# michal7kw/scRNA_seq_QAnnealing_Clustering

Measured on AMD Instinct MI355X. Metric: spin-flip updates/sec (node) + best QUBO energy vs neal, PBMC3k SNN, higher is better.
Workload: dtype f32

## Files before the change

scrna_seq_qannealing_clustering_amd/csrc/sparse_pair_kernels.hip:

```cpp
#include "mi_sa_device.h"

namespace mi_sa_impl {

namespace {

typedef _Float16 half_t;

#ifdef MI_K2P_PROFILE
#define K2P_TICK(var) do { asm volatile("s_waitcnt lgkmcnt(0)" ::: "memory"); const unsigned long long now_ = __builtin_amdgcn_s_memtime(); var += now_ - tick_; tick_ = now_; } while (0)
#else
#define K2P_TICK(var) do { } while (0)
#endif

__device__ __forceinline__ float half_lo(uint32_t w) { return (float)__builtin_bit_cast(half_t, (uint16_t)w); }
__device__ __forceinline__ float half_hi(uint32_t w) { return (float)__builtin_bit_cast(half_t, (uint16_t)(w >> 16)); }

template <int D, bool TW, bool WGT = false, int RW = D, int N16 = 0>
__global__ void __launch_bounds__(TW ? 128 : 64, TW ? 1 : 2) k_anneal_csr_rank1_pair(EllArgs a)
{
    static_assert(RW > D - 4 && RW <= D, "trimmed rows drop part of the last group of four only");
    static_assert(N16 == 0 || !WGT, "the weighted form keeps the 32-bit packing");
    static_assert(N16 != 2 || (TW && D == 16), "the pipelined unpack lives in the threshold-wavefront form's gather window");
    extern __shared__ __attribute__((aligned(16))) char lds[];
    const int lane = threadIdx.x & 63;
    const int pair = blockIdx.x;
    const int rA = 2 * pair, rB = 2 * pair + 1;
    if (rA >= a.R) return;
    const bool liveB = rB < a.R;
    const uint32_t gidA = a.replica_offset + (uint32_t)rA, gidB = gidA + 1u;
    const int n = a.n, slots = a.slots;
    const uint8_t *init = static_cast<const uint8_t *>(a.init);
    uint32_t *cell = reinterpret_cast<uint32_t *>(lds);
    const uint32_t ring_lane = (uint32_t)slots * 256u + (uint32_t)lane * 8u;

    if constexpr (TW) {
        if (__builtin_amdgcn_readfirstlane((int)(threadIdx.x >> 6)) == 1) {
            uint32_t wa[4], wb[4];
            uint32_t buf = 0;
            for (int s = 0; s < a.num_sweeps; ++s) {
                float TA, TB;
                if (a.temps_per_replica) {
                    TA = __int_as_float(__builtin_amdgcn_readfirstlane(__float_as_int(a.temps[rA])));
                    TB = __int_as_float(__builtin_amdgcn_readfirstlane(__float_as_int(a.temps[liveB ? rB : rA])));
                } else {
                    TA = TB = __int_as_float(__builtin_amdgcn_readfirstlane(__float_as_int(a.temps[s])));
                }
                const uint32_t sw = (uint32_t)s + a.sweep_offset;
#pragma unroll 1
                for (int t = 0; t < slots; t += 4) {
#ifdef MI_K2P_DBG_NOPROD
                    for (int c = 0; c < 4; ++c) wa[c] = wb[c] = (uint32_t)(t + c) * 0x9E3779B9u + lane * 77u;
#else
                    philox4x32_10((uint32_t)((t >> 2) * 64 + lane), sw, gidA, 0u, a.seed_lo, a.seed_hi, wa);
                    philox4x32_10((uint32_t)((t >> 2) * 64 + lane), sw, gidB, 0u, a.seed_lo, a.seed_hi, wb);
#endif
                    const uint32_t at = ring_lane + buf;
#pragma unroll
                    for (int c = 0; c < 4; ++c) {
                        const f32x2_t thr = neglog_u2(wa[c], wb[c]) * f32x2_t{TA, TB};
                        asm volatile("ds_write_b64 %0, %1 offset:%2" :: "v"(at), "v"(thr), "n"(c * 512) : "memory");
                    }
                    buf ^= 2048u;
                    asm volatile("s_waitcnt lgkmcnt(0)" ::: "memory");
                    __builtin_amdgcn_s_barrier();
                }
            }
            return;
        }
    }

    const int wslot = WGT ? a.wslot : -1;
    const int wl = wslot >= 0 ? a.wgt[lane] : 0;
    int SA = 0, SB = 0;
    for (int tg = 0; tg * 4 < slots; ++tg) {
        uint32_t wa[4] = {0u, 0u, 0u, 0u}, wb[4] = {0u, 0u, 0u, 0u};
        if (!init) {
            philox4x32_10((uint32_t)(tg * 64 + lane), 0u, gidA, 1u, a.seed_lo, a.seed_hi, wa);
            philox4x32_10((uint32_t)(tg * 64 + lane), 0u, gidB, 1u, a.seed_lo, a.seed_hi, wb);
        }
#pragma unroll
        for (int c = 0; c < 4; ++c) {
            const int t = 4 * tg + c;
            if (t >= slots) break;
            const int i = t * 64 + lane;
            bool xa, xb;
            const bool real = i < n && a.lin[i] < INFINITY;
            if (init) {
                xa = real && init[(size_t)rA * n + i] != 0;
                xb = real && liveB && init[(size_t)rB * n + i] != 0;
            } else {
                xa = real && (wa[c] >> 31);
                xb = real && (wb[c] >> 31);
            }
            cell[i] = (xa ? 0x3c00u : 0u) | (xb ? 0x3c000000u : 0u);
            if (WGT && t == wslot) {
                SA += (int)wave_sum_i64(xa ? (long long)wl : 0ll);
                SB += (int)wave_sum_i64(xb ? (long long)wl : 0ll);
            } else {
                SA += __popcll(__ballot(xa));
                SB += __popcll(__ballot(xb));
            }
        }
    }

    constexpr int G = D / 4;
    constexpr int LW = RW - 4 * (G - 1);
    constexpr int GC = N16 ? G / 2 : G;
    constexpr int SLOT_BYTES = N16 ? (GC + G) * 1024 : (G - 1) * 2048 + (LW == 3 ? 1792 : LW * 512);
    const __amdgpu_buffer_rsrc_t rs_adj = __builtin_amdgcn_make_buffer_rsrc(
        const_cast<uint4 *>(a.adj4), 0, slots * SLOT_BYTES, 0x00020000);
    const __amdgpu_buffer_rsrc_t rs_lin = __builtin_amdgcn_make_buffer_rsrc(
        const_cast<float *>(a.lin), 0, slots * 256, 0x00020000);
    struct SlotAdj { u32x4 col[GC]; u32x4 val[G]; uint32_t lin; };
    struct NbrPack { u32x4 w[GC]; };
    const int lane16 = lane * 16;
    auto fetch_block16 = [&](int t, int b) {
        const int tt = t < slots ? t : slots - 1;
        return __builtin_amdgcn_raw_buffer_load_b128(rs_adj, lane16 + (b & 3) * 1024, tt * SLOT_BYTES + (b >> 2) * 4096, 0);
    };
    auto fetch_nbr16 = [&](int t) {
        NbrPack q;
#pragma unroll
        for (int b = 0; b < GC; ++b) q.w[b] = fetch_block16(t, b);
        return q;
    };
    auto fetch_val16 = [&](int t) {
        SlotAdj p;
#pragma unroll
        for (int g = 0; g < G; ++g) p.val[g] = fetch_block16(t, GC + g);
        if constexpr (RW < D) p.lin = p.val[G - 1][3];
        else p.lin = __builtin_amdgcn_raw_buffer_load_b32(rs_lin, lane * 4, (t < slots ? t : slots - 1) * 256, 0);
        return p;
    };
    uint32_t m16 = 0xffffu;
    asm("" : "+s"(m16));
    auto unpack16 = [&](const u32x4 *w, int e) -> uint32_t {
        const uint32_t pw = w[e / 8][(e / 2) & 3];
        return (e & 1) ? pw >> 16 : (pw & m16);
    };
    uint32_t addr[16];
#ifdef MI_K2P_NOFETCH
    auto fetch_real = [&](int t) {
#else
    auto fetch_adj = [&](int t) {
#endif
        if constexpr (N16 != 0) {
            SlotAdj p = fetch_val16(t);
            const NbrPack q = fetch_nbr16(t);
#pragma unroll
            for (int b = 0; b < GC; ++b) p.col[b] = q.w[b];
            return p;
        }
        SlotAdj p;
        const int tt = t < slots ? t : slots - 1;
        const int soff = tt * SLOT_BYTES;
#pragma unroll
        for (int g = 0; g < G; ++g) {
            const int so = soff + (g / 2) * 4096, io = (g & 1) * 2048;
            if (LW == 4 || g < G - 1) {
                p.col[g] = __builtin_amdgcn_raw_buffer_load_b128(rs_adj, lane16 + io, so, 0);
                p.val[g] = __builtin_amdgcn_raw_buffer_load_b128(rs_adj, lane16 + io + 1024, so, 0);
            } else if constexpr (LW == 3) {
                p.col[g] = __builtin_amdgcn_raw_buffer_load_b128(rs_adj, lane16 + io, so, 0);
                const u32x2 v = __builtin_amdgcn_raw_buffer_load_b64(rs_adj, lane * 8 + io + 1024, so, 0);
                p.val[g] = u32x4{v.x, v.y, __builtin_amdgcn_raw_buffer_load_b32(rs_adj, lane * 4 + io + 1536, so, 0), 0u};
            } else if constexpr (LW == 2) {
                const u32x2 c = __builtin_amdgcn_raw_buffer_load_b64(rs_adj, lane * 8 + io, so, 0);
                const u32x2 v = __builtin_amdgcn_raw_buffer_load_b64(rs_adj, lane * 8 + io + 512, so, 0);
                p.col[g] = __builtin_shufflevector(c, c, 0, 1, -1, -1);
                p.val[g] = __builtin_shufflevector(v, v, 0, 1, -1, -1);
            } else {
                p.col[g][0] = __builtin_amdgcn_raw_buffer_load_b32(rs_adj, lane * 4 + io, so, 0);
                p.val[g][0] = __builtin_amdgcn_raw_buffer_load_b32(rs_adj, lane * 4 + io + 256, so, 0);
            }
        }
        if constexpr (LW == 3) p.lin = p.col[G - 1][3];
        else p.lin = __builtin_amdgcn_raw_buffer_load_b32(rs_lin, lane * 4, tt * 256, 0);
        return p;
    };
#ifdef MI_K2P_NOFETCH
    const SlotAdj adj0 = fetch_real(0);
    auto fetch_adj = [&](int) { return adj0; };
#endif

#ifdef MI_K2P_PROFILE
    unsigned long long tick_ = __builtin_amdgcn_s_memtime(), t_top = 0, t_gather = 0, t_sum = 0, t_rounds = 0, t_barrier = 0;
#endif
#ifndef MI_K2P_DBG_NOPRIO
    if constexpr (TW) __builtin_amdgcn_s_setprio(3);
#endif
    unsigned long long accepted = 0;
    uint32_t accA = 0, accB = 0;
    uint32_t wa[4] = {0u, 0u, 0u, 0u}, wb[4] = {0u, 0u, 0u, 0u};
    float TA = 1.0f, TB = 1.0f;
    const float cp = a.c_pair;
    uint32_t ring_buf = 0u;

    auto slot_body = [&](auto c_in_group, int t, const SlotAdj &cur, NbrPack &nxt, uint32_t wordA, uint32_t wordB) {
        constexpr int C = decltype(c_in_group)::value;
        const int i = t * 64 + lane;
        uint32_t own;
        float gA = __uint_as_float(cur.lin), gB = gA;
        float thrA = 0.0f, thrB = 0.0f;
        f32x2_t thr2 = {0.0f, 0.0f};
        uint32_t xiA = 0u, xiB = 0u, sgA = 0u, sgB = 0u;
        uint64_t XA = 0ull, XB = 0ull;
        f32x2_t cs = {0.0f, 0.0f}, csf = {0.0f, 0.0f};
        int ownA = 0, ownB = 0;
        auto own_terms = [&]() {
            xiA = (own >> 13) & 1u;
            xiB = own >> 29;
            XA = __ballot((own & 0xffffu) != 0u);
            XB = __ballot((own >> 16) != 0u);
            sgA = xiA << 31;
            sgB = xiB << 31;
            cs = f32x2_t{__uint_as_float(__float_as_uint(cp) ^ sgA), __uint_as_float(__float_as_uint(cp) ^ sgB)};
            ownA = SA - (int)xiA;
            ownB = SB - (int)xiB;
            csf = cs * f32x2_t{(float)ownA, (float)ownB};
        };
        K2P_TICK(t_top);
#pragma unroll
        for (int g0 = 0; g0 < G; g0 += 4) {
            constexpr int NK0 = RW < 16 ? RW : 16;
            const int NK = g0 == 0 ? NK0 : (RW - 4 * g0 < 16 ? RW - 4 * g0 : 16);
            uint32_t word[16];
            if (g0 == 0) asm volatile("ds_read_b32 %0, %1" : "=v"(own) : "v"(i * 4));
            if (g0 == 0 && TW) asm volatile("ds_read_b64 %0, %1 offset:%2" : "=v"(thr2) : "v"(ring_lane + ring_buf), "n"(C * 512));
#pragma unroll
            for (int k = 0; k < 16; ++k)
                if (k < NK)
#ifdef MI_K2P_DBG_LINEAR
                asm volatile("ds_read_b32 %0, %1" : "=v"(word[k]) : "v"((cur.col[g0 + k / 4][k & 3] & 0x3f00u) + lane * 4));
#else
                {
                    if constexpr (N16 == 2) asm volatile("ds_read_b32 %0, %1" : "=v"(word[k]) : "v"(addr[k]));
                    else if constexpr (N16 == 1) asm volatile("ds_read_b32 %0, %1" : "=v"(word[k]) : "v"(unpack16(cur.col, 4 * g0 + k)));
                    else
                asm volatile("ds_read_b32 %0, %1" : "=v"(word[k]) : "v"(cur.col[g0 + k / 4][k & 3]));
                }
#endif
            if (g0 == 0 && TW) {
                if constexpr (N16 == 2)
                    asm volatile("s_waitcnt lgkmcnt(%4)" : "+v"(own), "+v"(thr2), "+v"(nxt.w[0]), "+v"(nxt.w[1]) : "n"(NK0 < 15 ? NK0 : 15) : "memory");
                else
                asm volatile("s_waitcnt lgkmcnt(%2)" : "+v"(own), "+v"(thr2) : "n"(NK0 < 15 ? NK0 : 15) : "memory");
#ifndef MI_K2P_DBG_TERMS_AFTER
                own_terms();
#endif
                if constexpr (N16 == 2) {
#pragma unroll
                    for (int k = 0; k < NK0; ++k) {
                        addr[k] = unpack16(nxt.w, k);
                        asm volatile("" : "+v"(addr[k]));
                    }
                }
                asm volatile("s_waitcnt lgkmcnt(0)"
                             : "+v"(word[0]), "+v"(word[1]), "+v"(word[2]), "+v"(word[3]), "+v"(word[4]), "+v"(word[5]),
                               "+v"(word[6]), "+v"(word[7]), "+v"(word[8]), "+v"(word[9]), "+v"(word[10]), "+v"(word[11]),
                               "+v"(word[12]), "+v"(word[13]), "+v"(word[14]), "+v"(word[15]), "+v"(csf)
                             :: "memory");
                thrA = thr2.x;
                thrB = thr2.y;
            } else if (g0 == 0) {
                asm volatile("" : "+v"(wordA), "+v"(wordB));
                const f32x2_t thr = neglog_u2(wordA, wordB) * f32x2_t{TA, TB};
                thrA = thr.x;
                thrB = thr.y;
                asm volatile("s_waitcnt lgkmcnt(0)"
                             : "+v"(word[0]), "+v"(word[1]), "+v"(word[2]), "+v"(word[3]), "+v"(word[4]), "+v"(word[5]),
                               "+v"(word[6]), "+v"(word[7]), "+v"(word[8]), "+v"(word[9]), "+v"(word[10]), "+v"(word[11]),
                               "+v"(word[12]), "+v"(word[13]), "+v"(word[14]), "+v"(word[15]), "+v"(own), "+v"(thrA), "+v"(thrB)
                             :: "memory");
            } else {
                asm volatile("s_waitcnt lgkmcnt(0)"
                             : "+v"(word[0]), "+v"(word[1]), "+v"(word[2]), "+v"(word[3]), "+v"(word[4]), "+v"(word[5]),
                               "+v"(word[6]), "+v"(word[7]), "+v"(word[8]), "+v"(word[9]), "+v"(word[10]), "+v"(word[11]),
                               "+v"(word[12]), "+v"(word[13]), "+v"(word[14]), "+v"(word[15])
                             :: "memory");
            }
            K2P_TICK(t_gather);
#pragma unroll
            for (int k = 0; k < NK; ++k) {
                const float v = __uint_as_float(cur.val[g0 + k / 4][k & 3]);
                gA = __builtin_fmaf(v, half_lo(word[k]), gA);
                gB = __builtin_fmaf(v, half_hi(word[k]), gB);
            }
        }
#ifdef MI_K2P_DBG_TERMS_AFTER
        own_terms();
#else
        if constexpr (!TW) own_terms();
#endif
        if (WGT && t == wslot) {
            const uint64_t FA = weighted_slot_sweep(gA, thrA, wl, cp, xiA, SA, lane);
            const uint64_t FB = weighted_slot_sweep(gB, thrB, wl, cp, xiB, SB, lane);
            accA += (uint32_t)__popcll(FA);
            accB += (uint32_t)__popcll(FB);
            uint32_t fA, fB;
            asm("v_cndmask_b32 %0, 0, %1, %2" : "=v"(fA) : "v"(0x3c00u), "s"(FA));
            asm("v_cndmask_b32 %0, 0, %1, %2" : "=v"(fB) : "v"(0x3c000000u), "s"(FB));
            cell[i] = own ^ fA ^ fB;
            K2P_TICK(t_rounds);
            return;
        }
        const f32x2_t gs = {__uint_as_float(__float_as_uint(gA) ^ sgA), __uint_as_float(__float_as_uint(gB) ^ sgB)};
        f32x2_t de = gs + csf;
        bool mA = de.x < thrA, mB = de.y < thrB;
        uint64_t AA = __ballot(mA), AB = __ballot(mB);
        K2P_TICK(t_sum);
        if ((AA | AB) != 0ull) {
            const int baseA = ownA - (int)__builtin_amdgcn_mbcnt_hi((uint32_t)(XA >> 32), __builtin_amdgcn_mbcnt_lo((uint32_t)XA, 0u));
            const int baseB = ownB - (int)__builtin_amdgcn_mbcnt_hi((uint32_t)(XB >> 32), __builtin_amdgcn_mbcnt_lo((uint32_t)XB, 0u));
            uint64_t BA = AA ^ XA, BB = AB ^ XB;
#ifndef MI_K2P_DBG_NOROUNDS
#pragma nounroll
            for (;;) {
                const int sA = (int)__builtin_amdgcn_mbcnt_hi((uint32_t)(BA >> 32), __builtin_amdgcn_mbcnt_lo((uint32_t)BA, (uint32_t)baseA));
                const int sB = (int)__builtin_amdgcn_mbcnt_hi((uint32_t)(BB >> 32), __builtin_amdgcn_mbcnt_lo((uint32_t)BB, (uint32_t)baseB));
                de = gs + cs * f32x2_t{(float)sA, (float)sB};
                const uint64_t NBA = __ballot(de.x < thrA) ^ XA, NBB = __ballot(de.y < thrB) ^ XB;
                uint64_t d0 = NBA ^ BA, d1 = NBB ^ BB;
                asm("" : "+s"(d0), "+s"(d1));
                BA = NBA;
                BB = NBB;
                if ((d0 | d1) == 0ull) break;
            }
#endif
            AA = BA ^ XA;
            AB = BB ^ XB;
            SA += __popcll(BA) - __popcll(XA);
            SB += __popcll(BB) - __popcll(XB);
            accA += (uint32_t)__popcll(AA);
            accB += (uint32_t)__popcll(AB);
            uint32_t tA, tB;
            asm("v_cndmask_b32 %0, 0, %1, %2" : "=v"(tA) : "v"(0x3c00u), "s"(AA));
            asm("v_cndmask_b32 %0, 0, %1, %2" : "=v"(tB) : "v"(0x3c000000u), "s"(AB));
            cell[i] = own ^ tA ^ tB;
        }
        K2P_TICK(t_rounds);
    };

    using std::integral_constant;
    for (int s = 0; s < a.num_sweeps; ++s) {
        if constexpr (!TW) {
            if (a.temps_per_replica) {
                TA = __int_as_float(__builtin_amdgcn_readfirstlane(__float_as_int(a.temps[rA])));
                TB = __int_as_float(__builtin_amdgcn_readfirstlane(__float_as_int(a.temps[liveB ? rB : rA])));
            } else {
                TA = TB = __int_as_float(__builtin_amdgcn_readfirstlane(__float_as_int(a.temps[s])));
            }
        }
        const uint32_t sw = (uint32_t)s + a.sweep_offset;
        if constexpr (N16 == 2) {
            SlotAdj P = fetch_val16(0), Q;
            NbrPack NA = fetch_nbr16(0), NB;
#pragma unroll
            for (int k = 0; k < (RW < 16 ? RW : 16); ++k) addr[k] = unpack16(NA.w, k);
            NA = fetch_nbr16(1);
#pragma unroll 1
            for (int t = 0; t < slots; t += 4) {
                K2P_TICK(t_top);
                __builtin_amdgcn_s_barrier();
                K2P_TICK(t_barrier);
                Q = fetch_val16(t + 1);
                NB = fetch_nbr16(t + 2);
                slot_body(integral_constant<int, 0>{}, t, P, NA, wa[0], wb[0]);
                if (t + 1 < slots) {
                    P = fetch_val16(t + 2);
                    NA = fetch_nbr16(t + 3);
                    slot_body(integral_constant<int, 1>{}, t + 1, Q, NB, wa[1], wb[1]);
                    if (t + 2 < slots) {
                        Q = fetch_val16(t + 3);
                        NB = fetch_nbr16(t + 4);
                        slot_body(integral_constant<int, 2>{}, t + 2, P, NA, wa[2], wb[2]);
                        P = fetch_val16(t + 4);
                        NA = fetch_nbr16(t + 5);
                        if (t + 3 < slots) slot_body(integral_constant<int, 3>{}, t + 3, Q, NB, wa[3], wb[3]);
                    }
                }
                ring_buf ^= 2048u;
            }
        } else {
            NbrPack none;
            SlotAdj P = fetch_adj(0), Q;
    #pragma unroll 1
            for (int t = 0; t < slots; t += 4) {
                if constexpr (TW) {
                    K2P_TICK(t_top);
                    __builtin_amdgcn_s_barrier();
                    K2P_TICK(t_barrier);
                } else {
                    philox4x32_10((uint32_t)((t >> 2) * 64 + lane), sw, gidA, 0u, a.seed_lo, a.seed_hi, wa);
                    philox4x32_10((uint32_t)((t >> 2) * 64 + lane), sw, gidB, 0u, a.seed_lo, a.seed_hi, wb);
                }
                Q = fetch_adj(t + 1);
                slot_body(integral_constant<int, 0>{}, t, P, none, wa[0], wb[0]);
                if (t + 1 < slots) {
                    P = fetch_adj(t + 2);
                    slot_body(integral_constant<int, 1>{}, t + 1, Q, none, wa[1], wb[1]);
                    if (t + 2 < slots) {
                        Q = fetch_adj(t + 3);
                        slot_body(integral_constant<int, 2>{}, t + 2, P, none, wa[2], wb[2]);
                        P = fetch_adj(t + 4);
                        if (t + 3 < slots) slot_body(integral_constant<int, 3>{}, t + 3, Q, none, wa[3], wb[3]);
                    }
                }
                if constexpr (TW) ring_buf ^= 2048u;
            }
        }
        accepted += (unsigned long long)accA + (liveB ? (unsigned long long)accB : 0ull);
        accA = accB = 0;
    }

#pragma unroll 1
    for (int rep = 0; rep < 2; ++rep) {
        if (rep == 1 && !liveB) break;
        const int r = rep ? rB : rA;
        const int sh = rep ? 16 : 0;
        uint8_t *dst = static_cast<uint8_t *>(a.states) + (size_t)r * n;
        long long cnt = 0, cnt2 = 0;
        double e = 0.0;
        for (int t = 0; t < slots; ++t) {
            const int i = t * 64 + lane;
            const bool on = ((cell[i] >> sh) & 0xffffu) != 0u;
            if (i < n) dst[i] = (uint8_t)on;
            if (WGT && t == wslot) {
                cnt += wave_sum_i64(on ? (long long)wl : 0ll);
                cnt2 += wave_sum_i64(on ? (long long)wl * wl : 0ll);
            } else {
                const int c1 = __popcll(__ballot(on));
                cnt += c1;
                cnt2 += c1;
            }
            if (!on) continue;
            double acc = 0.0;
            for (int k = 0; k < D; ++k) {
                const size_t at = ((size_t)t * D + k) * 64 + lane;
                const uint32_t cc = a.ell_col[at];
                const double vv = a.ell_val64 ? a.ell_val64[at] : (double)a.ell_val[at];
                if (((cell[cc] >> sh) & 0xffffu) != 0u) acc += vv;
            }
            e += (a.lin64 ? a.lin64[i] : (double)a.lin[i]) + 0.5 * acc;
        }
        e = wave_sum_f64(e);
        if (lane == 0) {
            const double cp64 = a.ell_val64 ? a.c_pair64 : (double)a.c_pair;
            a.energy[r] = e + cp64 * 0.5 * ((double)cnt * (double)cnt - (double)cnt2) + a.offset;
        }
    }
    if (lane == 0) atomicAdd(&a.stats[1], accepted);
#ifdef MI_K2P_PROFILE
    if (lane == 0) {
        atomicAdd(&a.stats[8], t_top); atomicAdd(&a.stats[9], t_gather); atomicAdd(&a.stats[10], t_sum);
        atomicAdd(&a.stats[11], t_rounds); atomicAdd(&a.stats[12], t_barrier);
    }
#endif
}

}

int mi_launch_csr_rank1_pair(const EllArgs &a, const AnnealPlan &plan, hipStream_t st)
{
    if (!a.adj4) return fail(MI_EHIP, "csr_rank1 pair kernel: packed adjacency missing");
#ifdef MI_K2P_NOFETCH
    if (plan.nbr16) return fail(MI_EUNSUPPORTED, "the timing builds are arms of the 32-bit packing: set k2_nbr16 = 2");
#endif
    const int rw = plan.trim_rw ? plan.trim_rw : plan.D;
#define MI_K2P(D_, TW_, WGT_, RW_, N16_) \
    if (plan.D == D_ && plan.tw == TW_ && plan.weighted == WGT_ && rw == RW_ && (plan.nbr16 ? N16_ != 0 : N16_ == 0)) \
        return launch_planned(k_anneal_csr_rank1_pair<D_, TW_, WGT_, RW_, N16_>, a, plan, st);
    MI_K2P(16, true, true, 16, 0) MI_K2P(16, false, true, 16, 0)
    MI_K2P(16, true, false, 15, 2) MI_K2P(16, true, false, 14, 2) MI_K2P(16, true, false, 13, 2)
    MI_K2P(16, true, false, 15, 0) MI_K2P(16, true, false, 14, 0) MI_K2P(16, true, false, 13, 0)
    MI_K2P(16, true, false, 16, 2) MI_K2P(32, false, false, 32, 1)
    MI_K2P(16, true, false, 16, 0) MI_K2P(16, false, false, 16, 0) MI_K2P(32, false, false, 32, 0)
#undef MI_K2P
    return fail(MI_EUNSUPPORTED, "csr_rank1 pair kernel: slot-ELL width %d not built", a.D);
}

}
```

Baseline: 500.9 billion.

## Prefetch next slot's adjacency inside slot body and wrap prefetch across sweeps

In the 16-bit-packed pipelined path, the loads for upcoming slots are moved out of the outer loop and into each slot body via a callback, issued just before the LDS wait. The prefetch index wraps around to slot zero, so the pipeline carries into the next sweep without a per-sweep prologue refill. LDS cell and threshold-ring addresses become running base registers with immediate offsets, replacing per-slot address arithmetic. This adds state carried across sweeps and parity-dependent buffer swapping, which could be wrong for some slot counts.

```diff
diff --git a/scrna_seq_qannealing_clustering_amd/csrc/sparse_pair_kernels.hip b/scrna_seq_qannealing_clustering_amd/csrc/sparse_pair_kernels.hip
--- a/scrna_seq_qannealing_clustering_amd/csrc/sparse_pair_kernels.hip
+++ b/scrna_seq_qannealing_clustering_amd/csrc/sparse_pair_kernels.hip
@@ -114,9 +114,8 @@
     struct SlotAdj { u32x4 col[GC]; u32x4 val[G]; uint32_t lin; };
     struct NbrPack { u32x4 w[GC]; };
     const int lane16 = lane * 16;
-    auto fetch_block16 = [&](int t, int b) {
-        const int tt = t < slots ? t : slots - 1;
-        return __builtin_amdgcn_raw_buffer_load_b128(rs_adj, lane16 + (b & 3) * 1024, tt * SLOT_BYTES + (b >> 2) * 4096, 0);
+    auto fetch_block16 = [&](int w, int b) {
+        return __builtin_amdgcn_raw_buffer_load_b128(rs_adj, lane16 + (b & 3) * 1024, w * SLOT_BYTES + (b >> 2) * 4096, 0);
     };
     auto fetch_nbr16 = [&](int t) {
         NbrPack q;
@@ -129,7 +128,7 @@
 #pragma unroll
         for (int g = 0; g < G; ++g) p.val[g] = fetch_block16(t, GC + g);
         if constexpr (RW < D) p.lin = p.val[G - 1][3];
-        else p.lin = __builtin_amdgcn_raw_buffer_load_b32(rs_lin, lane * 4, (t < slots ? t : slots - 1) * 256, 0);
+        else p.lin = __builtin_amdgcn_raw_buffer_load_b32(rs_lin, lane * 4, t * 256, 0);
         return p;
     };
     uint32_t m16 = 0xffffu;
@@ -145,8 +144,9 @@
     auto fetch_adj = [&](int t) {
 #endif
         if constexpr (N16 != 0) {
-            SlotAdj p = fetch_val16(t);
-            const NbrPack q = fetch_nbr16(t);
+            const int tt = t < slots ? t : slots - 1;
+            SlotAdj p = fetch_val16(tt);
+            const NbrPack q = fetch_nbr16(tt);
 #pragma unroll
             for (int b = 0; b < GC; ++b) p.col[b] = q.w[b];
             return p;
@@ -195,8 +195,11 @@
     float TA = 1.0f, TB = 1.0f;
     const float cp = a.c_pair;
     uint32_t ring_buf = 0u;
-
-    auto slot_body = [&](auto c_in_group, int t, const SlotAdj &cur, NbrPack &nxt, uint32_t wordA, uint32_t wordB) {
+    uint32_t cellb = (uint32_t)lane * 4u;
+    uint32_t ringb = ring_lane;
+
+    using std::integral_constant;
+    auto slot_body = [&](auto c_in_group, int t, const SlotAdj &cur, NbrPack &nxt, uint32_t wordA, uint32_t wordB, auto &&prefetch) {
         constexpr int C = decltype(c_in_group)::value;
         const int i = t * 64 + lane;
         uint32_t own;
@@ -225,8 +228,13 @@
             constexpr int NK0 = RW < 16 ? RW : 16;
             const int NK = g0 == 0 ? NK0 : (RW - 4 * g0 < 16 ? RW - 4 * g0 : 16);
             uint32_t word[16];
+            if constexpr (N16 == 2) {
+                asm volatile("ds_read_b32 %0, %1 offset:%2" : "=v"(own) : "v"(cellb), "n"(C * 256));
+                asm volatile("ds_read_b64 %0, %1 offset:%2" : "=v"(thr2) : "v"(ringb), "n"(C * 512));
+            } else {
             if (g0 == 0) asm volatile("ds_read_b32 %0, %1" : "=v"(own) : "v"(i * 4));
             if (g0 == 0 && TW) asm volatile("ds_read_b64 %0, %1 offset:%2" : "=v"(thr2) : "v"(ring_lane + ring_buf), "n"(C * 512));
+            }
 #pragma unroll
             for (int k = 0; k < 16; ++k)
                 if (k < NK)
@@ -241,6 +249,7 @@
                 }
 #endif
             if (g0 == 0 && TW) {
+                if constexpr (N16 == 2) prefetch();
                 if constexpr (N16 == 2)
                     asm volatile("s_waitcnt lgkmcnt(%4)" : "+v"(own), "+v"(thr2), "+v"(nxt.w[0]), "+v"(nxt.w[1]) : "n"(NK0 < 15 ? NK0 : 15) : "memory");
                 else
@@ -336,12 +345,40 @@
             uint32_t tA, tB;
             asm("v_cndmask_b32 %0, 0, %1, %2" : "=v"(tA) : "v"(0x3c00u), "s"(AA));
             asm("v_cndmask_b32 %0, 0, %1, %2" : "=v"(tB) : "v"(0x3c000000u), "s"(AB));
+            if constexpr (N16 == 2)
+                asm volatile("ds_write_b32 %0, %1 offset:%2" :: "v"(cellb), "v"(own ^ tA ^ tB), "n"(C * 256) : "memory");
+            else
             cell[i] = own ^ tA ^ tB;
         }
         K2P_TICK(t_rounds);
     };
 
-    using std::integral_constant;
+    SlotAdj P16, Q16;
+    NbrPack NA16, NB16;
+    int pfv = 0, pfn = 0;
+    auto prologue16 = [&]() {
+        P16 = fetch_val16(0);
+        NA16 = fetch_nbr16(0);
+#pragma unroll
+        for (int k = 0; k < (RW < 16 ? RW : 16); ++k) addr[k] = unpack16(NA16.w, k);
+        pfv = slots - 1 < 1 ? slots - 1 : 1;
+        const int two = slots - 1 < 2 ? slots - 1 : 2;
+        pfn = 2 * (two - pfv);
+        NA16 = fetch_nbr16(pfv);
+    };
+    auto prefetch16 = [&](SlotAdj &V, NbrPack &W) {
+        int w = pfn, u = pfv;
+        asm volatile("" : "+s"(w));
+        W = fetch_nbr16(w);
+        asm volatile("" : "+s"(u));
+        V = fetch_val16(u);
+        pfv = pfn;
+        pfn = pfn + 1 == slots ? 0 : pfn + 1;
+    };
+    auto pf_q = [&]() { prefetch16(Q16, NB16); };
+    auto pf_p = [&]() { prefetch16(P16, NA16); };
+    auto pf_none = []() {};
+    if constexpr (N16 == 2) prologue16();
     for (int s = 0; s < a.num_sweeps; ++s) {
         if constexpr (!TW) {
             if (a.temps_per_replica) {
@@ -353,33 +390,28 @@
         }
         const uint32_t sw = (uint32_t)s + a.sweep_offset;
         if constexpr (N16 == 2) {
-            SlotAdj P = fetch_val16(0), Q;
-            NbrPack NA = fetch_nbr16(0), NB;
-#pragma unroll
-            for (int k = 0; k < (RW < 16 ? RW : 16); ++k) addr[k] = unpack16(NA.w, k);
-            NA = fetch_nbr16(1);
 #pragma unroll 1
             for (int t = 0; t < slots; t += 4) {
                 K2P_TICK(t_top);
                 __builtin_amdgcn_s_barrier();
                 K2P_TICK(t_barrier);
-                Q = fetch_val16(t + 1);
-                NB = fetch_nbr16(t + 2);
-                slot_body(integral_constant<int, 0>{}, t, P, NA, wa[0], wb[0]);
+                slot_body(integral_constant<int, 0>{}, t, P16, NA16, wa[0], wb[0], pf_q);
                 if (t + 1 < slots) {
-                    P = fetch_val16(t + 2);
-                    NA = fetch_nbr16(t + 3);
-                    slot_body(integral_constant<int, 1>{}, t + 1, Q, NB, wa[1], wb[1]);
+                    slot_body(integral_constant<int, 1>{}, t + 1, Q16, NB16, wa[1], wb[1], pf_p);
                     if (t + 2 < slots) {
-                        Q = fetch_val16(t + 3);
-                        NB = fetch_nbr16(t + 4);
-                        slot_body(integral_constant<int, 2>{}, t + 2, P, NA, wa[2], wb[2]);
-                        P = fetch_val16(t + 4);
-                        NA = fetch_nbr16(t + 5);
-                        if (t + 3 < slots) slot_body(integral_constant<int, 3>{}, t + 3, Q, NB, wa[3], wb[3]);
+                        slot_body(integral_constant<int, 2>{}, t + 2, P16, NA16, wa[2], wb[2], pf_q);
+                        if (t + 3 < slots) slot_body(integral_constant<int, 3>{}, t + 3, Q16, NB16, wa[3], wb[3], pf_p);
                     }
                 }
                 ring_buf ^= 2048u;
+                cellb += 1024u;
+                ringb = ring_lane + ring_buf;
+                asm volatile("" : "+v"(cellb), "+v"(ringb));
+            }
+            cellb = (uint32_t)lane * 4u;
+            if (slots & 1) {
+                P16 = Q16;
+                NA16 = NB16;
             }
         } else {
             NbrPack none;
@@ -395,15 +427,15 @@
                     philox4x32_10((uint32_t)((t >> 2) * 64 + lane), sw, gidB, 0u, a.seed_lo, a.seed_hi, wb);
                 }
                 Q = fetch_adj(t + 1);
-                slot_body(integral_constant<int, 0>{}, t, P, none, wa[0], wb[0]);
+                slot_body(integral_constant<int, 0>{}, t, P, none, wa[0], wb[0], pf_none);
                 if (t + 1 < slots) {
                     P = fetch_adj(t + 2);
-                    slot_body(integral_constant<int, 1>{}, t + 1, Q, none, wa[1], wb[1]);
+                    slot_body(integral_constant<int, 1>{}, t + 1, Q, none, wa[1], wb[1], pf_none);
                     if (t + 2 < slots) {
                         Q = fetch_adj(t + 3);
-                        slot_body(integral_constant<int, 2>{}, t + 2, P, none, wa[2], wb[2]);
+                        slot_body(integral_constant<int, 2>{}, t + 2, P, none, wa[2], wb[2], pf_none);
                         P = fetch_adj(t + 4);
-                        if (t + 3 < slots) slot_body(integral_constant<int, 3>{}, t + 3, Q, none, wa[3], wb[3]);
+                        if (t + 3 < slots) slot_body(integral_constant<int, 3>{}, t + 3, Q, none, wa[3], wb[3], pf_none);
                     }
                 }
                 if constexpr (TW) ring_buf ^= 2048u;
```

Result: faster. 508.3 billion, median of 6 (+1.5%).
